# Nuralamsiddik16/Ultrafnd_git

Hardware: AMD Instinct MI355X
Metric: train-step samples/sec (FakeSV batch, seq128+224^2) (higher is better)
Workload: dtype bf16

## Files before the change

### ultrafnd_git_amd/csrc/gemm_bf16_kernel.hpp

```cpp
#pragma once
#ifndef UFND_GEMM_OUT_NT
#define UFND_GEMM_OUT_NT 0
#endif

#include <type_traits>

#include "common.hpp"
#include "attn_softmax.hpp"

#pragma clang fp contract(off)

#ifndef UFND_GEMM_ILV
#define UFND_GEMM_ILV 1
#endif

namespace {

constexpr int BK = 64;

struct GemmArgs {
  const __bf16* A;
  const __bf16* W;
  const float* bias;
  const float* residual;
  __bf16* out_bf16;
  float* out_f32;
  int M, N, K, lda, ldw, ldr, ldo, ldf, act;
  int m_tiles, n_tiles;
  unsigned long long* stamps;
  const float* a_stats;
  const float* colsum;
  const float* r_stats;
  const float* r_gamma;
  const float* r_beta;
  float* out_stats;
  int a_parts, r_parts;
  float a_eps, r_eps, inv_h;
  const int32_t* att_mask;
  __bf16* att_ctx;
  int att_h;
  int xcd_cols;
  float att_scale_log2e;
  const __bf16* residual_b;
  int ldrb;
  int ksplit;
  size_t slab_stride;
  const __bf16* aux;
  int ldaux;
  float* guard;
  int pp_rows;
  const int* m_live;
  const int32_t* att_cu;
  const int32_t* att_bins;
  const int* att_nbins;
};

__device__ __forceinline__ void dma16(const void* gsrc, void* lds_dst) {
  __builtin_amdgcn_global_load_lds((const void __attribute__((address_space(1)))*)gsrc,
                                   (void __attribute__((address_space(3)))*)lds_dst, 16, 0, 0);
}

__device__ __forceinline__ float opaque_f(float x) {
  asm volatile("" : "+v"(x));
  return x;
}
__device__ __forceinline__ f32x2 opaque_f2(f32x2 x) {
  asm volatile("" : "+v"(x));
  return x;
}

__device__ __forceinline__ bf16x8 lds_frag(const char* tile, int row, int chunk) {
  return *reinterpret_cast<const bf16x8*>(tile + row * 128 + ((chunk ^ ((row >> 1) & 7)) << 4));
}

template <int N>
__device__ __forceinline__ void wait_vmcnt() {
  static_assert(N >= 0 && N <= 63, "vmcnt range");
  asm volatile("s_waitcnt vmcnt(%0)" ::"n"(N) : "memory");
}

template <int V> struct IntC { static constexpr int value = V; };

constexpr int gemm_waves_per_simd(int BM, int BN, int WM, int WN, int STA, int STB, int MI, int LNX, int ATT) {
  const int ring = (STA * BM + STB * BN) * 128, cbytes = WM * WN * MI * (BN / WN + 4) * 4;
  const int smem = (ring > cbytes ? ring : cbytes) + (LNX ? BM * 8 + 64 : 0);
  return (!ATT && smem <= 80 * 1024 ? 2 : 1) * WM * WN / 4;
}
template <int BM, int BN, int WM, int WN, int STA, int STB, int MI, int ABL = 0, int DBG = 0, int LNX = 0, int ATT = 0, int BWD = 0>
__global__ __launch_bounds__(WM * WN * 64) __attribute__((amdgpu_waves_per_eu(gemm_waves_per_simd(BM, BN, WM, WN, STA, STB, MI, LNX, ATT))))
void gemm_bf16_kernel(const GemmArgs a) {
  static_assert(!BWD || (!LNX && !ATT && !ABL && !DBG), "backward forms are plain kernels");
  static_assert(MI == 16 || MI == 32, "MFMA shape");
  static_assert(!ATT || (BM == 128 && BN == 384 && MI == 16 && WM * WN == 8 && LNX == 1), "fused attention tile");
  using acc_t = typename std::conditional<MI == 16, f32x4, f32x16>::type;
  constexpr int AR = MI * MI / 64;
  constexpr int KQ = MI == 16 ? 1 : 2;
  constexpr int NW = WM * WN;
  constexpr int TM = BM / WM, TN = BN / WN;
  constexpr int MT = TM / MI, NT = TN / MI;
  constexpr int ASLOT = BM * 128, BSLOT = BN * 128;
  constexpr int DA = STA - 1, DB = STB - 1;
  constexpr int APIECES = BM / 8, BPIECES = BN / 8;
  constexpr int PWA = APIECES / NW, PWB = (BPIECES + NW - 1) / NW;
  constexpr int WAITN = PWA * (DA - 1 > 0 ? DA - 1 : 0) + PWB * (DB - 1 > 0 ? DB - 1 : 0);
  constexpr int CP = TN + 4;
  constexpr int CBYTES = NW * MI * CP * 4;
  constexpr int RING = STA * ASLOT + STB * BSLOT;
  constexpr int ATT_OFF = (CBYTES + 1023) & ~1023;
  constexpr int ATT_END = ATT ? ATT_OFF + 6 * 16384 + 2048 : 0;
  constexpr int STAT_OFF0 = (RING > CBYTES) ? RING : CBYTES;
  constexpr int STAT_OFF = STAT_OFF0 > ATT_END ? STAT_OFF0 : ATT_END;
  constexpr int SMEM = STAT_OFF + (LNX ? BM * 8 + 64 : 0);
  static_assert(SMEM <= 160 * 1024, "LDS budget");
  static_assert(APIECES % NW == 0 && TM % MI == 0 && TN % MI == 0, "tile split");
  static_assert(STB >= 2 && (STA == STB || STA == STB + 1), "ring depths");
  static_assert(WAITN <= 63, "vmcnt range");
  __shared__ __attribute__((aligned(16))) char smem[SMEM];

  unsigned long long stamp[10];
  if constexpr (DBG) {
    stamp[0] = __builtin_amdgcn_s_memtime();
    stamp[1] = __builtin_amdgcn_s_memrealtime();
  }

  int mlive = a.M, m_tiles = a.m_tiles;
  if constexpr (!BWD && !ATT) {
    if (a.m_live) {
      const int v = __builtin_amdgcn_readfirstlane(*a.m_live);
      mlive = v < a.M ? (v > 0 ? v : 0) : a.M;
      m_tiles = (mlive + BM - 1) / BM;
      if ((int)blockIdx.x >= m_tiles * a.n_tiles) return;
    }
  }
  if constexpr (ATT) {
    if (a.att_bins) {
      const int v = __builtin_amdgcn_readfirstlane(*a.att_nbins);
      m_tiles = v < a.m_tiles ? (v > 0 ? v : 0) : a.m_tiles;
      if ((int)blockIdx.x >= m_tiles * a.n_tiles) return;
    }
  }
  const int nblk = m_tiles * a.n_tiles;
  int bid, kslice = 0;
  {
    const int ngrid = BWD ? nblk * (a.ksplit > 1 ? a.ksplit : 1) : nblk;
    const int q = ngrid >> 3, r = ngrid & 7, xcd = blockIdx.x & 7, idx = blockIdx.x >> 3;
    bid = (xcd < r ? xcd * (q + 1) : r * (q + 1) + (xcd - r) * q) + idx;
    if constexpr (BWD) {
      kslice = bid / nblk;
      bid -= kslice * nblk;
    }
  }
  int tm = bid / a.n_tiles, tn = bid % a.n_tiles;
  if (a.xcd_cols == 2) {
    const int nh = a.n_tiles >> 1, per_half = m_tiles * nh;
    const int half = bid / per_half, rem = bid - half * per_half;
    tm = rem / nh;
    tn = half * nh + (rem - tm * nh);
  }
  const int m0 = tm * BM, n0 = tn * BN;
  int arow0 = m0, alen = BM;
  int srow[4] = {0, 0, 0, 0}, scnt[4] = {0, 0, 0, 0}, smeta[4] = {-1, -1, -1, -1};
  const bool slots = ATT && a.att_bins != nullptr;
  if constexpr (ATT) {
    if (slots) {
      const int32_t* bd = a.att_bins + (size_t)tm * 8;
#pragma unroll
      for (int j = 0; j < 4; ++j) {
        srow[j] = __builtin_amdgcn_readfirstlane(bd[2 * j]);
        smeta[j] = __builtin_amdgcn_readfirstlane(bd[2 * j + 1]);
        const int n = smeta[j] & 255, rest = n - 32 * ((smeta[j] >> 8) & 3);
        scnt[j] = smeta[j] < 0 ? 0 : (rest < 32 ? rest : 32);
      }
#pragma unroll
      for (int j = 1; j < 4; ++j) srow[j] = scnt[j] > 0 ? srow[j] : srow[0];
    } else if (a.att_cu) {
      mlive = __builtin_amdgcn_readfirstlane(*a.m_live);
      arow0 = __builtin_amdgcn_readfirstlane(a.att_cu[tm]);
      alen = __builtin_amdgcn_readfirstlane(a.att_cu[tm + 1]) - arow0;
      if (alen <= 0) return;
    }
  } else {
    alen = mlive - m0;
  }
  auto tile_row = [&](int tr) {
    if (slots) {
      const int j = tr >> 5, q = tr & 31;
      const int r0 = j == 0 ? srow[0] : j == 1 ? srow[1] : j == 2 ? srow[2] : srow[3];
      const int c = j == 0 ? scnt[0] : j == 1 ? scnt[1] : j == 2 ? scnt[2] : scnt[3];
      return r0 + (q < c ? q : (c > 0 ? c - 1 : 0));
    }
    const int gr = arow0 + tr;
    return gr < mlive ? gr : mlive - 1;
  };
  auto tile_row_live = [&](int tr) {
    if (slots) {
      const int j = tr >> 5;
      return (tr & 31) < (j == 0 ? scnt[0] : j == 1 ? scnt[1] : j == 2 ? scnt[2] : scnt[3]);
    }
    return tr < alen;
  };
  const int wave = __builtin_amdgcn_readfirstlane(threadIdx.x >> 6), lane = threadIdx.x & 63;
  const int wm = wave / WN, wn = wave % WN, fr = lane & (MI - 1), g = lane / MI;

  acc_t acc[MT][NT];
#pragma unroll
  for (int i = 0; i < MT; ++i)
#pragma unroll
    for (int j = 0; j < NT; ++j)
#pragma unroll
      for (int r = 0; r < AR; ++r) acc[i][j][r] = 0.f;

  int nk = a.K / BK, kbase = 0;
  if constexpr (BWD) {
    if (a.ksplit > 1) {
      const int per = (nk + a.ksplit - 1) / a.ksplit;
      kbase = kslice * per * BK;
      nk = nk - kslice * per < per ? nk - kslice * per : per;
    }
  }
  const int prow = lane >> 3, ppos = lane & 7;
  int arow_att[ATT ? PWA : 1];
  if constexpr (ATT) {
#pragma unroll
    for (int ii = 0; ii < PWA; ++ii) arow_att[ii] = tile_row(8 * (wave + NW * ii) + prow);
  }
  auto issueA = [&](int t, int kt) {
    char* buf = smem + (t % STA) * ASLOT;
    const int k0 = kbase + kt * BK;
#pragma unroll
    for (int ii = 0; ii < PWA; ++ii) {
      const int p = wave + NW * ii;
      const int r = 8 * p + prow;
      const int c = ppos ^ ((r >> 1) & 7);
      int gr = arow0 + r;
      gr = gr < mlive ? gr : mlive - 1;
      if constexpr (ATT) gr = arow_att[ii];
      dma16(a.A + (size_t)gr * a.lda + k0 + c * 8, buf + p * 1024);
    }
  };
  auto issueB = [&](int t, int kt) {
    char* buf = smem + STA * ASLOT + (t % STB) * BSLOT;
    const int k0 = kbase + kt * BK;
#pragma unroll
    for (int ii = 0; ii < PWB; ++ii) {
      int p = wave + NW * ii;
      if constexpr (BPIECES % NW != 0) p = p < BPIECES ? p : p - BPIECES;
      const int r = 8 * p + prow;
      const int c = ppos ^ ((r >> 1) & 7);
      int gr = n0 + r;
      gr = gr < a.N ? gr : a.N - 1;
      if constexpr (ATT) gr = (r >> 7) * a.att_h + tn * 128 + (r & 127);
      dma16(a.W + (size_t)gr * a.ldw + k0 + c * 8, buf + p * 1024);
    }
  };
  constexpr int TPR = NW * 64 / BM;
  static_assert(!LNX || TPR == 2 || TPR == 4, "threads per tile row");
  constexpr int GPT = 4 / (TPR < 4 ? TPR : 4);
  f32x4 sv[GPT][3];
  f32x2* st_lds = reinterpret_cast<f32x2*>(smem + STAT_OFF);
  const float* sp = nullptr;
  if constexpr (LNX) {
    sp = a.a_stats ? a.a_stats : a.r_stats;
    if (sp) {
      const int parts = a.a_stats ? a.a_parts : a.r_parts;
      int row = arow0 + (int)threadIdx.x / TPR;
      row = row < mlive ? row : mlive - 1;
      if constexpr (ATT) row = tile_row((int)threadIdx.x / TPR);
      const f32x4* base = reinterpret_cast<const f32x4*>(sp + (size_t)row * parts * 2);
      const int nq = parts >> 1, sub = threadIdx.x % TPR;
#pragma unroll
      for (int gi = 0; gi < GPT; ++gi)
#pragma unroll
        for (int u = 0; u < 3; ++u) {
          const int q = (sub + gi * TPR) + 4 * u;
          asm volatile("global_load_dwordx4 %0, %1, off" : "=v"(sv[gi][u]) : "v"(base + (q < nq ? q : 0)) : "memory");
        }
    }
  }
  int att_mk = 1;
  if constexpr (ATT) {
    if (slots) {
      const int j = (int)threadIdx.x >> 7, k = threadIdx.x & 127;
      const int mt = j == 0 ? smeta[0] : j == 1 ? smeta[1] : j == 2 ? smeta[2] : smeta[3];
      att_mk = mt >= 0 && k < (mt & 255);
      if (att_mk && a.att_mask) att_mk = a.att_mask[(size_t)(mt >> 10) * BM + k];
    } else if (a.att_mask && threadIdx.x < BM) {
      att_mk = a.att_mask[m0 + threadIdx.x];
    }
  }
#pragma unroll
  for (int s = 0; s < STA; ++s) {
    const int ks = s < nk ? s : nk - 1;
    if (s < STB && (LNX || s < nk)) issueB(s, ks);
    if (LNX || s < nk) issueA(s, ks);
  }

  if constexpr (LNX) {
    if (sp) {
      constexpr int NPRO = STA * PWA + STB * PWB;
      static_assert(NPRO <= 63, "vmcnt range");
      if constexpr (GPT == 1)
        asm volatile("s_waitcnt vmcnt(%3) ; STATRETIRE %0 %1 %2" : "+v"(sv[0][0]), "+v"(sv[0][1]), "+v"(sv[0][2]) : "n"(NPRO) : "memory");
      else
        asm volatile("s_waitcnt vmcnt(%6) ; STATRETIRE %0 %1 %2 %3 %4 %5" : "+v"(sv[0][0]), "+v"(sv[0][1]), "+v"(sv[0][2]), "+v"(sv[GPT - 1][0]),
                     "+v"(sv[GPT - 1][1]), "+v"(sv[GPT - 1][2]) : "n"(NPRO) : "memory");
      const int nq_ = (a.a_stats ? a.a_parts : a.r_parts) >> 1, sub_ = threadIdx.x % TPR;
      float gs[GPT], gq[GPT];
#pragma unroll
      for (int gi = 0; gi < GPT; ++gi) {
#pragma unroll
        for (int u = 0; u < 3; ++u) {
          if ((sub_ + gi * TPR) + 4 * u >= nq_) sv[gi][u] = f32x4{0.f, 0.f, 0.f, 0.f};
        }
        gs[gi] = sv[gi][0][0] + sv[gi][0][2];
        gq[gi] = sv[gi][0][1] + sv[gi][0][3];
#pragma unroll
        for (int u = 1; u < 3; ++u) { gs[gi] += sv[gi][u][0] + sv[gi][u][2]; gq[gi] += sv[gi][u][1] + sv[gi][u][3]; }
      }
      float sm, sq;
      if constexpr (TPR == 4) {
        sm = gs[0] + quad_xor1(gs[0]);
        sq = gq[0] + quad_xor1(gq[0]);
        sm += quad_xor2(sm);
        sq += quad_xor2(sq);
      } else {
        const float s01 = gs[0] + quad_xor1(gs[0]), s23 = gs[1] + quad_xor1(gs[1]);
        const float q01 = gq[0] + quad_xor1(gq[0]), q23 = gq[1] + quad_xor1(gq[1]);
        sm = s01 + s23;
        sq = q01 + q23;
      }
      const float mean = __fmul_rn(sm, a.inv_h);
      const float var = fmaxf(__fmaf_rn(-mean, mean, __fmul_rn(sq, a.inv_h)), 0.f);
      const float rstd = __builtin_amdgcn_rsqf(__fadd_rn(var, a.a_stats ? a.a_eps : a.r_eps));
      if (threadIdx.x % TPR == 0) st_lds[threadIdx.x / TPR] = f32x2{mean, rstd};
      if (a.guard && a.a_stats) {
        float ratio = __fmul_rn(fabsf(mean), rstd);
        ratio = ratio == ratio ? ratio : INFINITY;
        const float worst = wave_max(threadIdx.x % TPR == 0 && tile_row_live((int)threadIdx.x / TPR) ? ratio : 0.0f);
        if (lane == 0) reinterpret_cast<float*>(smem + STAT_OFF + BM * 8)[wave] = worst;
      }
      asm volatile("s_waitcnt lgkmcnt(0)" ::: "memory");
    }
  }

  bf16x8 af0[KQ][MT], bf0[KQ][NT], af1[KQ][MT], bf1[KQ][NT];
  auto read_half = [&](int t, auto kk_, bf16x8 (&af)[KQ][MT], bf16x8 (&bfr)[KQ][NT]) {
    constexpr int kk = decltype(kk_)::value;
    const char* At = smem + (t % STA) * ASLOT;
    const char* Bt = smem + STA * ASLOT + (t % STB) * BSLOT;
#pragma unroll
    for (int q = 0; q < KQ; ++q) {
      const int chunk = MI == 16 ? g + 4 * kk : g + 2 * q + 4 * kk;
#pragma unroll
      for (int i = 0; i < MT; ++i) af[q][i] = lds_frag(At, wm * TM + i * MI + fr, chunk);
#pragma unroll
      for (int j = 0; j < NT; ++j) bfr[q][j] = lds_frag(Bt, wn * TN + j * MI + fr, chunk);
    }
  };
  auto mma_half = [&](const bf16x8 (&af)[KQ][MT], const bf16x8 (&bfr)[KQ][NT]) {
#pragma unroll
    for (int q = 0; q < KQ; ++q)
#pragma unroll
      for (int i = 0; i < MT; ++i)
#pragma unroll
        for (int j = 0; j < NT; ++j) {
          if constexpr (MI == 16) acc[i][j] = __builtin_amdgcn_mfma_f32_16x16x32_bf16(af[q][i], bfr[q][j], acc[i][j], 0, 0, 0);
          else acc[i][j] = __builtin_amdgcn_mfma_f32_32x32x16_bf16(af[q][i], bfr[q][j], acc[i][j], 0, 0, 0);
        }
  };
  constexpr int NMF = KQ * MT * NT, NRD = KQ * (MT + NT);
  constexpr bool ILV = UFND_GEMM_ILV != 0;
  auto body = [&](int t, auto ia_, auto ib_, auto next_) {
    constexpr bool IA = decltype(ia_)::value != 0, IB = decltype(ib_)::value != 0, NEXT = decltype(next_)::value != 0;
    if constexpr (ABL != 1) {
      read_half(t, IntC<1>{}, af1, bf1);
      mma_half(af0, bf0);
      if constexpr (ILV) {
#pragma unroll
        for (int q = 0; q < (NRD < NMF ? NRD : NMF - 1); ++q) {
          __builtin_amdgcn_sched_group_barrier(0x008, 1, 0);
          __builtin_amdgcn_sched_group_barrier(0x100, 1, 0);
        }
        __builtin_amdgcn_sched_group_barrier(0x100, NRD - (NRD < NMF ? NRD : NMF - 1), 0);
        __builtin_amdgcn_sched_group_barrier(0x008, NMF - (NRD < NMF ? NRD : NMF - 1), 0);
      } else {
        __builtin_amdgcn_sched_group_barrier(0x008, 1, 0);
        __builtin_amdgcn_sched_group_barrier(0x100, NRD, 0);
        __builtin_amdgcn_sched_group_barrier(0x008, NMF - 1, 0);
      }
    }
    if constexpr (NEXT) {
      __builtin_amdgcn_sched_barrier(0);
      if (t + STA - 1 < nk) wait_vmcnt<WAITN>();
      else wait_vmcnt<0>();
      asm volatile("s_waitcnt lgkmcnt(0)" ::: "memory");
      __builtin_amdgcn_s_barrier();
      __builtin_amdgcn_sched_barrier(0);
      if constexpr (ABL != 1) read_half(t + 1, IntC<0>{}, af0, bf0);
      if constexpr (ABL != 2) {
        if constexpr (IB) issueB(t + STB, t + STB);
        if constexpr (IA) issueA(t + STA, t + STA);
      }
    }
    if constexpr (ABL != 1) {
      mma_half(af1, bf1);
      constexpr int PW = (ABL == 2 || !NEXT) ? 0 : (IA ? PWA : 0) + (IB ? PWB : 0);
      constexpr int GRP = (NMF - 1) / (PW + 1) > 0 ? (NMF - 1) / (PW + 1) : 1;
      if constexpr (ILV && NEXT && NRD + PW < NMF) {
#pragma unroll
        for (int q = 0; q < NRD; ++q) {
          __builtin_amdgcn_sched_group_barrier(0x008, 1, 0);
          __builtin_amdgcn_sched_group_barrier(0x100, 1, 0);
        }
        constexpr int REST = NMF - NRD, G2 = REST / (PW + 1) > 0 ? REST / (PW + 1) : 1;
#pragma unroll
        for (int q = 0; q < PW; ++q) {
          __builtin_amdgcn_sched_group_barrier(0x008, G2, 0);
          __builtin_amdgcn_sched_group_barrier(0x020, 1, 0);
        }
        __builtin_amdgcn_sched_group_barrier(0x008, REST - G2 * PW > 0 ? REST - G2 * PW : 0, 0);
      } else {
        __builtin_amdgcn_sched_group_barrier(0x008, 1, 0);
        if constexpr (NEXT) __builtin_amdgcn_sched_group_barrier(0x100, NRD, 0);
#pragma unroll
        for (int q = 0; q < PW; ++q) {
          __builtin_amdgcn_sched_group_barrier(0x008, GRP, 0);
          __builtin_amdgcn_sched_group_barrier(0x020, 1, 0);
        }
        __builtin_amdgcn_sched_group_barrier(0x008, NMF - 1 - GRP * PW > 0 ? NMF - 1 - GRP * PW : 0, 0);
      }
    }
  };

  if (STA <= nk) wait_vmcnt<PWA * (STA - 1) + PWB * (STB - 1)>();
  else wait_vmcnt<0>();
  __builtin_amdgcn_sched_barrier(0);
  __builtin_amdgcn_s_barrier();
  __builtin_amdgcn_sched_barrier(0);
  if constexpr (DBG) {
    stamp[2] = __builtin_amdgcn_s_memtime();
    stamp[3] = __builtin_amdgcn_s_memrealtime();
  }
  if constexpr (ABL != 1) read_half(0, IntC<0>{}, af0, bf0);
  int t = 0;
  for (; t + STA < nk; ++t) body(t, IntC<1>{}, IntC<1>{}, IntC<1>{});
  for (; t + STB < nk; ++t) body(t, IntC<0>{}, IntC<1>{}, IntC<1>{});
  for (; t + 1 < nk; ++t) body(t, IntC<0>{}, IntC<0>{}, IntC<1>{});
  body(t, IntC<0>{}, IntC<0>{}, IntC<0>{});
  __builtin_amdgcn_sched_barrier(0);
  __builtin_amdgcn_s_barrier();
  __builtin_amdgcn_sched_barrier(0);
  if constexpr (DBG) {
    stamp[4] = __builtin_amdgcn_s_memtime();
    stamp[5] = __builtin_amdgcn_s_memrealtime();
  }

  float bj[NT], csj[NT];
#pragma unroll
  for (int j = 0; j < NT; ++j) { bj[j] = 0.f; csj[j] = 0.f; }
  auto gcol = [&](int c) { return ATT ? (c >> 7) * a.att_h + tn * 128 + (c & 127) : n0 + c; };
  if (a.bias) {
#pragma unroll
    for (int j = 0; j < NT; ++j) bj[j] = a.bias[gcol(wn * TN + j * MI + fr)];
  }
  bool fold = false, rln = false;
  if constexpr (LNX) {
    fold = a.a_stats != nullptr;
    rln = a.r_stats != nullptr;
    if (fold) {
#pragma unroll
      for (int j = 0; j < NT; ++j) csj[j] = a.colsum[gcol(wn * TN + j * MI + fr)];
    }
  }
  float* cst = reinterpret_cast<float*>(smem) + wave * MI * CP;
  float* const outf = (BWD && a.out_f32) ? a.out_f32 + (size_t)kslice * a.slab_stride : a.out_f32;
  constexpr int CPR = TN / 8;
  constexpr int CHUNKS = MI * CPR;
  constexpr int NIT = (CHUNKS + 63) / 64;
  constexpr bool FIXCOL = (64 % CPR) == 0;
  auto ld8 = [&](const float* ptr, float (&o)[8]) {
    const f32x4 x0 = *reinterpret_cast<const f32x4*>(ptr), x1 = *reinterpret_cast<const f32x4*>(ptr + 4);
#pragma unroll
    for (int q = 0; q < 4; ++q) { o[q] = x0[q]; o[4 + q] = x1[q]; }
  };
  float g8[8], b8[8];
  if constexpr (LNX && FIXCOL) {
    if (rln) {
      const int col = n0 + wn * TN + (lane % CPR) * 8;
      ld8(a.r_gamma + col, g8);
      ld8(a.r_beta + col, b8);
    }
  }
  auto epilogue = [&](auto act_, auto mode_) {
    constexpr int ACT = decltype(act_)::value;
    constexpr bool FOLD = LNX && decltype(mode_)::value == 1, RLN = LNX && decltype(mode_)::value == 2;
    constexpr bool RES = !FOLD;
#pragma unroll
    for (int i = 0; i < MT; ++i) {
      float rr8[RES ? NIT : 1][8];
      if constexpr (RES) if (a.residual && !(BWD && a.aux)) {
#pragma unroll
        for (int it = 0; it < NIT; ++it) {
          const int id = lane + 64 * it;
          if (id < CHUNKS) {
            int row = m0 + wm * TM + i * MI + id / CPR;
            row = row < a.M ? row : a.M - 1;
            ld8(a.residual + (size_t)row * a.ldr + n0 + wn * TN + (id % CPR) * 8, rr8[it]);
          }
        }
      }
      if constexpr (BWD) {
        if (a.aux) {
#pragma unroll
          for (int it = 0; it < NIT; ++it) {
            const int id = lane + 64 * it;
            if (id < CHUNKS) {
              int row = m0 + wm * TM + i * MI + id / CPR;
              row = row < a.M ? row : a.M - 1;
              const bf16x8 xb = *reinterpret_cast<const bf16x8*>(a.aux + (size_t)row * a.ldaux + n0 + wn * TN + (id % CPR) * 8);
#pragma unroll
              for (int q = 0; q < 8; ++q) rr8[it][q] = (float)xb[q];
            }
          }
        }
      }
      if constexpr (LNX && RES) {
        if (a.residual_b) {
#pragma unroll
          for (int it = 0; it < NIT; ++it) {
            const int id = lane + 64 * it;
            if (id < CHUNKS) {
              int row = m0 + wm * TM + i * MI + id / CPR;
              row = row < a.M ? row : a.M - 1;
              const bf16x8 rb = *reinterpret_cast<const bf16x8*>(a.residual_b + (size_t)row * a.ldrb + n0 + wn * TN + (id % CPR) * 8);
#pragma unroll
              for (int q = 0; q < 8; ++q) rr8[it][q] = (float)rb[q];
            }
          }
        }
      }
#pragma unroll
      for (int r = 0; r < AR; r += 2) {
        const int prow_ = MI == 16 ? 4 * g + r : 8 * (r >> 2) + 4 * g + (r & 3);
        f32x2 mean2 = {0.f, 0.f}, rstd2 = {1.f, 1.f};
        if constexpr (FOLD) {
          const f32x2 a0 = st_lds[wm * TM + i * MI + prow_], a1 = st_lds[wm * TM + i * MI + prow_ + 1];
          mean2 = f32x2{a0[0], a1[0]};
          rstd2 = f32x2{a0[1], a1[1]};
        }
#pragma unroll
        for (int j = 0; j < NT; ++j) {
          f32x2 v = {acc[i][j][r], acc[i][j][r + 1]};
          if constexpr (FOLD) v = opaque_f2(rstd2 * __builtin_elementwise_fma(-mean2, f32x2{csj[j], csj[j]}, v));
          v = v + f32x2{bj[j], bj[j]};
          if constexpr (ACT == UFND_ACT_GELU) v = gelu_fast_f2(v);
          else if constexpr (ACT == UFND_ACT_QUICK_GELU) v = quick_gelu_fast_f2(v);
          cst[prow_ * CP + j * MI + fr] = v.x;
          cst[(prow_ + 1) * CP + j * MI + fr] = v.y;
        }
      }
      asm volatile("s_waitcnt lgkmcnt(0)" ::: "memory");
#pragma unroll
      for (int it = 0; it < NIT; ++it) {
        const int id = lane + 64 * it;
        if (id >= CHUNKS) break;
        const int rr = id / CPR, cl = (id % CPR) * 8;
        const int row = m0 + wm * TM + i * MI + rr;
        const int col = n0 + wn * TN + cl;
        const bool live = row < mlive;
        const f32x4 v0 = *reinterpret_cast<const f32x4*>(cst + rr * CP + cl);
        const f32x4 v1 = *reinterpret_cast<const f32x4*>(cst + rr * CP + cl + 4);
        float v[8] = {v0[0], v0[1], v0[2], v0[3], v1[0], v1[1], v1[2], v1[3]};
        if constexpr (BWD) {
          if (a.aux) {
            if (a.act == UFND_ACT_GELU_BWD) {
#pragma unroll
              for (int q = 0; q < 8; ++q) v[q] = v[q] * gelu_grad_f(rr8[it][q]);
            } else {
#pragma unroll
              for (int q = 0; q < 8; ++q) v[q] = v[q] * quick_gelu_grad_f(rr8[it][q]);
            }
          }
        }
        if constexpr (RES) if ((a.residual && !(BWD && a.aux)) || (LNX && a.residual_b)) {
          if constexpr (RLN) {
            const f32x2 ms = st_lds[wm * TM + i * MI + rr];
            if constexpr (!FIXCOL) {
              ld8(a.r_gamma + col, g8);
              ld8(a.r_beta + col, b8);
            }
#pragma unroll
            for (int q = 0; q < 8; ++q) rr8[it][q] = __fmaf_rn(__fmul_rn(__fsub_rn(rr8[it][q], ms[0]), ms[1]), g8[q], b8[q]);
          }
#pragma unroll
          for (int q = 0; q < 8; ++q) v[q] = __fadd_rn(v[q], rr8[it][q]);
        }
        if constexpr (LNX && RES) {
          if (a.out_stats) {
            if constexpr (CPR % 4 == 0) {
              float sm = 0.f, sq = 0.f;
#pragma unroll
              for (int q = 0; q < 8; ++q) { sm = __fadd_rn(sm, v[q]); sq = __fmaf_rn(v[q], v[q], sq); }
              sm += quad_xor1(sm);
              sq += quad_xor1(sq);
              sm += quad_xor2(sm);
              sq += quad_xor2(sq);
              if (live && (id & 3) == 0)
                *reinterpret_cast<f32x2*>(a.out_stats + ((size_t)row * (a.N >> 5) + (col >> 5)) * 2) = f32x2{sm, sq};
            }
          }
        }
        if constexpr (ATT) {
          const int ct = wn * TN + cl;
          const int trow = wm * TM + i * MI + rr, img = ct >> 6, ch = (ct & 63) >> 3;
          bf16x8 o;
#pragma unroll
          for (int q = 0; q < 8; ++q) o[q] = (__bf16)v[q];
          const int sw = img >= 4 ? (ch ^ (((trow >> 1) & 3) << 1)) : (ch ^ ((trow >> 1) & 7));
          *reinterpret_cast<bf16x8*>(smem + ATT_OFF + img * 16384 + trow * 128 + (sw << 4)) = o;
          continue;
        }
        if (!live) continue;
        if (a.out_f32) {
          float* op = outf + (size_t)row * a.ldf + col;
          *reinterpret_cast<f32x4*>(op) = f32x4{v[0], v[1], v[2], v[3]};
          *reinterpret_cast<f32x4*>(op + 4) = f32x4{v[4], v[5], v[6], v[7]};
        }
        if (a.out_bf16) {
          bf16x8 o;
#pragma unroll
          for (int q = 0; q < 8; ++q) o[q] = (__bf16)v[q];
          if constexpr (UFND_GEMM_OUT_NT && !BWD) __builtin_nontemporal_store(o, reinterpret_cast<bf16x8*>(a.out_bf16 + (size_t)row * a.ldo + col));
          else *reinterpret_cast<bf16x8*>(a.out_bf16 + (size_t)row * a.ldo + col) = o;
        }
      }
      asm volatile("s_waitcnt lgkmcnt(0)" ::: "memory");
    }
  };
  if constexpr (LNX) {
    if (fold) {
      if (a.act == UFND_ACT_GELU) epilogue(IntC<UFND_ACT_GELU>{}, IntC<1>{});
      else if (a.act == UFND_ACT_QUICK_GELU) epilogue(IntC<UFND_ACT_QUICK_GELU>{}, IntC<1>{});
      else epilogue(IntC<UFND_ACT_NONE>{}, IntC<1>{});
    } else if (rln) {
      epilogue(IntC<UFND_ACT_NONE>{}, IntC<2>{});
    } else {
      epilogue(IntC<UFND_ACT_NONE>{}, IntC<0>{});
    }
  } else {
    if (a.act == UFND_ACT_GELU) epilogue(IntC<UFND_ACT_GELU>{}, IntC<0>{});
    else if (a.act == UFND_ACT_QUICK_GELU) epilogue(IntC<UFND_ACT_QUICK_GELU>{}, IntC<0>{});
    else epilogue(IntC<UFND_ACT_NONE>{}, IntC<0>{});
  }
  if constexpr (ATT && DBG) {
    stamp[8] = __builtin_amdgcn_s_memtime();
    stamp[9] = __builtin_amdgcn_s_memrealtime();
  }
  if constexpr (ATT) {
    constexpr float NEG_MASK = -3.0e38f;
    float* kbias = reinterpret_cast<float*>(smem + ATT_OFF + 6 * 16384);
    if (slots || threadIdx.x < BM) kbias[threadIdx.x] = att_mk != 0 ? 0.0f : NEG_MASK;
    __syncthreads();
    const int hh = wave >> 2, wq = wave & 3, g4 = lane >> 4, f16 = lane & 15;
    int wrow0 = arow0 + 32 * wq, wcnt = alen - 32 * wq, koff = 0;
    const float* wbias = kbias;
    if (slots) {
      const int mt = wq == 0 ? smeta[0] : wq == 1 ? smeta[1] : wq == 2 ? smeta[2] : smeta[3];
      wrow0 = wq == 0 ? srow[0] : wq == 1 ? srow[1] : wq == 2 ? srow[2] : srow[3];
      wcnt = wq == 0 ? scnt[0] : wq == 1 ? scnt[1] : wq == 2 ? scnt[2] : scnt[3];
      koff = 32 * (wq - ((mt >> 8) & 3));
      wbias = kbias + wq * BM;
    }
    const char* qimg = smem + ATT_OFF + hh * 16384;
    const char* kimg = smem + ATT_OFF + (2 + hh) * 16384;
    const char* vimg = smem + ATT_OFF + (4 + hh) * 16384;
    bf16x8 qf[2][2];
#pragma unroll
    for (int qt = 0; qt < 2; ++qt) {
      const int q = wq * 32 + qt * 16 + f16;
      qf[qt][0] = lds_frag(qimg, q, g4);
      qf[qt][1] = lds_frag(qimg, q, g4 + 4);
    }
    f32x4 o[4][2];
#pragma unroll
    for (int dt = 0; dt < 4; ++dt)
#pragma unroll
      for (int qt = 0; qt < 2; ++qt) o[dt][qt] = f32x4{0.f, 0.f, 0.f, 0.f};
    float m_run[2] = {-INFINITY, -INFINITY}, l_run[2] = {0.f, 0.f};
    constexpr int KB = 64, KT = KB / 16;
    if (wcnt > 0) {
#pragma unroll
    for (int kb0 = 0; kb0 < BM; kb0 += KB) {
      const int kr0 = koff + kb0;
      if (masked_block_is_noop(wbias + kb0, lane, m_run)) continue;
      f32x4 sc[KT][2];
#pragma unroll
      for (int kt = 0; kt < KT; ++kt)
#pragma unroll
        for (int qt = 0; qt < 2; ++qt) sc[kt][qt] = f32x4{0.f, 0.f, 0.f, 0.f};
#pragma unroll
      for (int kk = 0; kk < 2; ++kk)
#pragma unroll
        for (int kt = 0; kt < KT; ++kt) {
          const bf16x8 kf = lds_frag(kimg, (kr0 + kt * 16 + f16) & (BM - 1), g4 + 4 * kk);
#pragma unroll
          for (int qt = 0; qt < 2; ++qt) sc[kt][qt] = __builtin_amdgcn_mfma_f32_16x16x32_bf16(kf, qf[qt][kk], sc[kt][qt], 0, 0, 0);
        }
      const bool any_masked = __any(wbias[kb0 + lane] != 0.0f);
      bf16x8 pf[KT / 2][2];
#pragma unroll
      for (int qt = 0; qt < 2; ++qt) {
        const float alpha = online_softmax_block<KT>(sc, qt, wbias + kb0, any_masked, g4, a.att_scale_log2e, m_run[qt], l_run[qt], pf);
        if (!__all(alpha == 1.0f)) {
#pragma unroll
          for (int dt = 0; dt < 4; ++dt) o[dt][qt] *= alpha;
        }
      }
#pragma unroll
      for (int ksd = 0; ksd < KT / 2; ++ksd) {
#pragma unroll
        for (int dt = 0; dt < 4; ++dt) {
          const int qq = f16 >> 2, pp = f16 & 3;
          const int key0 = (kr0 + 32 * ksd + 4 * g4 + qq) & (BM - 1);
          const int ch = 2 * dt + (pp >> 1);
          const int off0 = key0 * 128 + ((ch ^ (((key0 >> 1) & 3) << 1)) << 4) + 8 * (pp & 1);
          const int key1 = key0 + 16;
          const int off1 = key1 * 128 + ((ch ^ (((key1 >> 1) & 3) << 1)) << 4) + 8 * (pp & 1);
          const s16x4 t0 = __builtin_amdgcn_ds_read_tr16_b64_v4i16((s16x4 __attribute__((address_space(3)))*)(vimg + off0));
          const s16x4 t1 = __builtin_amdgcn_ds_read_tr16_b64_v4i16((s16x4 __attribute__((address_space(3)))*)(vimg + off1));
          union { s16x4 s2[2]; bf16x8 v; } u;
          u.s2[0] = t0;
          u.s2[1] = t1;
#pragma unroll
          for (int qt = 0; qt < 2; ++qt) o[dt][qt] = __builtin_amdgcn_mfma_f32_16x16x32_bf16(u.v, pf[ksd][qt], o[dt][qt], 0, 0, 0);
        }
      }
    }
    }
#pragma unroll
    for (int qt = 0; qt < 2; ++qt) {
      float l = l_run[qt];
      l += __shfl_xor(l, 16, 64);
      l += __shfl_xor(l, 32, 64);
      const float inv = 1.0f / l;
      const int q = qt * 16 + f16;
      if (q >= wcnt) continue;
      __bf16* dst = a.att_ctx + (size_t)(wrow0 + q) * a.att_h + (tn * 2 + hh) * 64 + 4 * g4;
#pragma unroll
      for (int dt = 0; dt < 4; ++dt) {
        bf16x4 ov = {(__bf16)(o[dt][qt][0] * inv), (__bf16)(o[dt][qt][1] * inv), (__bf16)(o[dt][qt][2] * inv), (__bf16)(o[dt][qt][3] * inv)};
        *reinterpret_cast<bf16x4*>(dst + dt * 16) = ov;
      }
    }
  }
  if constexpr (LNX) {
    if (a.guard && a.a_stats && threadIdx.x == 0) {
      const float* gw = reinterpret_cast<const float*>(smem + STAT_OFF + BM * 8);
      float worst = gw[0];
#pragma unroll
      for (int w = 1; w < NW; ++w) worst = fmaxf(worst, gw[w]);
      atomicMax(reinterpret_cast<int*>(a.guard + (blockIdx.x & 1023)), __float_as_int(worst));
    }
  }
  if constexpr (DBG) {
    asm volatile("s_waitcnt vmcnt(0)" ::: "memory");
    stamp[6] = __builtin_amdgcn_s_memtime();
    stamp[7] = __builtin_amdgcn_s_memrealtime();
    if (threadIdx.x == 0) {
      constexpr int NS = ATT ? 10 : 8;
#pragma unroll
      for (int i = 0; i < NS; ++i) a.stamps[(size_t)blockIdx.x * NS + i] = stamp[i];
    }
  }
}

}

#define UFND_GEMM_TILES(X)                                                                             \
  X(0, 128, 128, 2, 2, 3, 3, 16, 0, 0)                                                              \
  X(1, 128, 64, 2, 2, 3, 3, 16, 0, 0)                                                 \
  X(2, 256, 128, 4, 2, 3, 3, 16, 1, 1)                                                              \
  X(3, 128, 128, 2, 2, 2, 2, 16, 1, 0)                                                \
  X(4, 128, 64, 2, 2, 4, 4, 16, 0, 0)                                                               \
  X(5, 256, 64, 4, 2, 3, 3, 16, 0, 0)                                                               \
  X(6, 128, 288, 2, 2, 3, 3, 16, 0, 0)                                   \
  X(7, 128, 96, 2, 2, 3, 3, 16, 0, 0)                                     \
  X(8, 256, 192, 4, 2, 2, 2, 16, 1, 1)                                  \
  X(9, 128, 384, 2, 2, 2, 2, 16, 0, 0)                                                              \
  X(10, 128, 192, 2, 2, 3, 3, 16, 0, 0)                                                             \
  X(11, 128, 96, 2, 2, 4, 4, 16, 0, 0)                                                              \
  X(12, 64, 96, 1, 2, 4, 4, 16, 0, 0)                     \
  X(13, 64, 192, 1, 2, 3, 3, 16, 0, 0)                                                              \
  X(14, 128, 256, 2, 2, 2, 2, 16, 0, 0)                                                             \
  X(15, 256, 256, 4, 2, 2, 2, 16, 1, 1)                                                             \
  X(16, 128, 128, 4, 2, 3, 3, 16, 1, 1)                                  \
  X(17, 128, 192, 4, 2, 3, 3, 16, 1, 1)                                  \
  X(18, 256, 64, 4, 2, 4, 4, 16, 0, 0)                                                              \
  X(19, 64, 64, 1, 2, 4, 4, 16, 0, 0)                                                 \
  X(20, 128, 64, 4, 2, 4, 4, 16, 1, 1)                                   \
  X(21, 256, 192, 2, 4, 2, 2, 16, 0, 0)                                          \
  X(22, 256, 192, 4, 2, 3, 2, 16, 1, 1)                                 \
  X(23, 256, 256, 4, 2, 3, 2, 16, 0, 0)                                                             \
  X(24, 128, 192, 4, 2, 4, 4, 16, 0, 0)                                                             \
  X(25, 128, 256, 4, 2, 3, 3, 16, 0, 0)                                 \
  X(26, 256, 192, 4, 2, 2, 2, 32, 0, 0)   \
  X(27, 128, 128, 4, 2, 3, 3, 32, 0, 0)                                                                    \
  X(28, 256, 144, 8, 1, 2, 2, 16, 1, 1)   \
  X(29, 128, 128, 4, 2, 2, 2, 16, 1, 0)

#ifdef UFND_DIAG
#define UFND_TILE_BUILT(PROD_) 1
#else
#define UFND_TILE_BUILT(PROD_) (PROD_)
#endif

struct TileCfg { int bm, bn, threads, wn, lnx, built; };
static const TileCfg kTiles[] = {
#define X(id, BM_, BN_, WM_, WN_, SA_, SB_, MI_, LN_, PROD_) {BM_, BN_, WM_ * WN_ * 64, WN_, LN_, UFND_TILE_BUILT(PROD_)},
    UFND_GEMM_TILES(X)
#undef X
};
constexpr int kNumTiles = sizeof(kTiles) / sizeof(kTiles[0]);

static int xcd_cols_for(int M, int N, int K, int m_tiles, int n_tiles) {
#ifdef UFND_DIAG
  static const int forced = [] { const char* e = getenv("UFND_GEMM_XCD_COLS"); return e ? atoi(e) : 0; }();
  if (forced == 1) return 1;
  if (forced == 2) return (n_tiles % 2 == 0) ? 2 : 1;
#endif
  (void)K;
  return (4LL * N > (long long)M && n_tiles % 2 == 0 && m_tiles >= 4) ? 2 : 1;
}

static int launch_cfg(int cfg, int mode, GemmArgs& a, hipStream_t stream) {
  if (cfg < 0 || cfg >= kNumTiles || !kTiles[cfg].built) {
    ufnd_set_error("gemm_bf16: tile config %d is not part of this library", cfg);
    return UFND_ERR_INVALID;
  }
  const TileCfg& t = kTiles[cfg];
  a.m_tiles = ufnd_cdiv(a.M, t.bm);
  a.n_tiles = a.N / t.bn;
  a.xcd_cols = xcd_cols_for(a.M, a.N, a.K, a.m_tiles, a.n_tiles);
  const dim3 grid(a.m_tiles * a.n_tiles * (mode == 6 && a.ksplit > 1 ? a.ksplit : 1)), block(t.threads);
#ifdef UFND_GEMM_ONLY_BWD
#define X(id, BM_, BN_, WM_, WN_, SA_, SB_, MI_, LN_, PROD_)                                                                      \
  case id:                                                                                                                        \
    if constexpr (id == 15 || id == 16 || id == 17 || id == 20 || id == 22) {                                                     \
      hipLaunchKernelGGL((gemm_bf16_kernel<BM_, BN_, WM_, WN_, SA_, SB_, MI_, 0, 0, 0, 0, 1>), grid, block, 0, stream, a);        \
    } else {                                                                                                                      \
      ufnd_set_error("gemm_bf16 backward: tile %d has no backward kernel", id);                                                   \
      return UFND_ERR_INVALID;                                                                                                    \
    }                                                                                                                             \
    break;
  (void)mode;
  switch (cfg) {
    UFND_GEMM_TILES(X)
    default: ufnd_set_error("gemm_bf16: unknown tile config %d", cfg); return UFND_ERR_INVALID;
  }
#undef X
  return UFND_OK;
#else
#ifdef UFND_DIAG
#define UFND_DIAG_LAUNCH(BM_, BN_, WM_, WN_, SA_, SB_, MI_)                                                                             \
  else if (mode == 5) hipLaunchKernelGGL((gemm_bf16_kernel<BM_, BN_, WM_, WN_, SA_, SB_, MI_, 0, 1, 1>), grid, block, 0, stream, a);   \
  else if (mode == 1) hipLaunchKernelGGL((gemm_bf16_kernel<BM_, BN_, WM_, WN_, SA_, SB_, MI_, 1, 0>), grid, block, 0, stream, a);      \
  else if (mode == 2) hipLaunchKernelGGL((gemm_bf16_kernel<BM_, BN_, WM_, WN_, SA_, SB_, MI_, 2, 0>), grid, block, 0, stream, a);      \
  else if (mode == 3) hipLaunchKernelGGL((gemm_bf16_kernel<BM_, BN_, WM_, WN_, SA_, SB_, MI_, 0, 1>), grid, block, 0, stream, a);
#else
#define UFND_DIAG_LAUNCH(BM_, BN_, WM_, WN_, SA_, SB_, MI_)
#endif
#define X(id, BM_, BN_, WM_, WN_, SA_, SB_, MI_, LN_, PROD_)                                                        \
  case id:                                                                                                          \
    if constexpr (UFND_TILE_BUILT(PROD_) != 0) {                                                                    \
      if (mode == 0) {                                                                                              \
        hipLaunchKernelGGL((gemm_bf16_kernel<BM_, BN_, WM_, WN_, SA_, SB_, MI_, 0, 0>), grid, block, 0, stream, a); \
      } else if constexpr (LN_ != 0) {    \
        if (mode == 4) hipLaunchKernelGGL((gemm_bf16_kernel<BM_, BN_, WM_, WN_, SA_, SB_, MI_, 0, 0, 1>), grid, block, 0, stream, a); \
        UFND_DIAG_LAUNCH(BM_, BN_, WM_, WN_, SA_, SB_, MI_)                                                         \
        else {                                                                                                      \
          ufnd_set_error("gemm_bf16: tile %d has no kernel for mode %d in this library", id, mode);                 \
          return UFND_ERR_INVALID;                                                                                  \
        }                                                                                                           \
      } else {                                                                                                      \
        ufnd_set_error("gemm_bf16: tile %d has no diagnostics / LayerNorm-aware build", id);                        \
        return UFND_ERR_INVALID;                                                                                    \
      }                                                                                                             \
    }                                                                                                               \
    break;
  switch (cfg) {
    UFND_GEMM_TILES(X)
    default: ufnd_set_error("gemm_bf16: unknown tile config %d", cfg); return UFND_ERR_INVALID;
  }
#undef X
#undef UFND_DIAG_LAUNCH
  return UFND_OK;
#endif
}

static int auto_cfg(int M, int N, int K) {
#ifdef UFND_DIAG
  static const int forced = [] { const char* e = getenv("UFND_GEMM_FORCE_CFG"); return e ? atoi(e) : -1; }();
  if (forced >= 0 && forced < kNumTiles && N % kTiles[forced].bn == 0) return forced;
#endif
  auto tiles = [&](int cfg) { return (long long)ufnd_cdiv(M, kTiles[cfg].bm) * (N / kTiles[cfg].bn); };
  if (N % 256 == 0 && N >= 3072 && tiles(15) >= 512) return 15;
  if (N % 256 == 0 && N >= 2048 && tiles(15) >= 190 && tiles(15) <= 256) return 15;
  if (N % 192 == 0 && tiles(22) >= 160) return 22;
  if (N >= 2048) {
    if (N % 192 == 0 && N >= 3072) return 17;
    if (N % 128 == 0) return 16;
  }
  if (N < 2048 && N % 192 == 0 && tiles(17) >= 150 && tiles(17) <= 256) return 17;
  if (N % 128 == 0 && tiles(16) >= 150) return 16;
  return 20;
}
```

Measured before the change: 29020.

## Write fused-attention QKV tiles from registers with V stored transposed in LDS

For the fused attention tile, the QKV GEMM epilogue now writes Q/K directly from MFMA accumulators (using swapped operand order so rows are contiguous) and stores V pre-transposed into a dedicated LDS image, instead of staging through the generic per-wave C buffer. The P·V loop then reads V fragments with plain 128-bit LDS loads instead of two ds_read_tr16 transposing reads per fragment. Column mapping per wave is changed so each wave owns head-aligned slices, and the attention region now overlaps the start of LDS. This removes a staging pass and the transpose-read cost but changes layout invariants in several places, with risk of aliasing the staging/ring regions.

```diff
diff --git a/ultrafnd_git_amd/csrc/gemm_bf16_kernel.hpp b/ultrafnd_git_amd/csrc/gemm_bf16_kernel.hpp
--- a/ultrafnd_git_amd/csrc/gemm_bf16_kernel.hpp
+++ b/ultrafnd_git_amd/csrc/gemm_bf16_kernel.hpp
@@ -106,7 +106,7 @@
   constexpr int CP = TN + 4;
   constexpr int CBYTES = NW * MI * CP * 4;
   constexpr int RING = STA * ASLOT + STB * BSLOT;
-  constexpr int ATT_OFF = (CBYTES + 1023) & ~1023;
+  constexpr int ATT_OFF = 0;
   constexpr int ATT_END = ATT ? ATT_OFF + 6 * 16384 + 2048 : 0;
   constexpr int STAT_OFF0 = (RING > CBYTES) ? RING : CBYTES;
   constexpr int STAT_OFF = STAT_OFF0 > ATT_END ? STAT_OFF0 : ATT_END;
@@ -202,6 +202,7 @@
   const int wave = __builtin_amdgcn_readfirstlane(threadIdx.x >> 6), lane = threadIdx.x & 63;
   const int wm = wave / WN, wn = wave % WN, fr = lane & (MI - 1), g = lane / MI;
 
+  auto wcol = [&](int j) { return ATT ? (j >> 1) * 128 + (2 * wn + (j & 1)) * MI : wn * TN + j * MI; };
   acc_t acc[MT][NT];
 #pragma unroll
   for (int i = 0; i < MT; ++i)
@@ -354,7 +355,7 @@
 #pragma unroll
       for (int i = 0; i < MT; ++i) af[q][i] = lds_frag(At, wm * TM + i * MI + fr, chunk);
 #pragma unroll
-      for (int j = 0; j < NT; ++j) bfr[q][j] = lds_frag(Bt, wn * TN + j * MI + fr, chunk);
+      for (int j = 0; j < NT; ++j) bfr[q][j] = lds_frag(Bt, wcol(j) + fr, chunk);
     }
   };
   auto mma_half = [&](const bf16x8 (&af)[KQ][MT], const bf16x8 (&bfr)[KQ][NT]) {
@@ -364,7 +365,10 @@
       for (int i = 0; i < MT; ++i)
 #pragma unroll
         for (int j = 0; j < NT; ++j) {
-          if constexpr (MI == 16) acc[i][j] = __builtin_amdgcn_mfma_f32_16x16x32_bf16(af[q][i], bfr[q][j], acc[i][j], 0, 0, 0);
+          if constexpr (ATT) {
+            if (j < 4) acc[i][j] = __builtin_amdgcn_mfma_f32_16x16x32_bf16(bfr[q][j], af[q][i], acc[i][j], 0, 0, 0);
+            else acc[i][j] = __builtin_amdgcn_mfma_f32_16x16x32_bf16(af[q][i], bfr[q][j], acc[i][j], 0, 0, 0);
+          } else if constexpr (MI == 16) acc[i][j] = __builtin_amdgcn_mfma_f32_16x16x32_bf16(af[q][i], bfr[q][j], acc[i][j], 0, 0, 0);
           else acc[i][j] = __builtin_amdgcn_mfma_f32_32x32x16_bf16(af[q][i], bfr[q][j], acc[i][j], 0, 0, 0);
         }
   };
@@ -459,7 +463,7 @@
 #pragma unroll
   for (int j = 0; j < NT; ++j) { bj[j] = 0.f; csj[j] = 0.f; }
   auto gcol = [&](int c) { return ATT ? (c >> 7) * a.att_h + tn * 128 + (c & 127) : n0 + c; };
-  if (a.bias) {
+  if (!ATT && a.bias) {
 #pragma unroll
     for (int j = 0; j < NT; ++j) bj[j] = a.bias[gcol(wn * TN + j * MI + fr)];
   }
@@ -467,7 +471,7 @@
   if constexpr (LNX) {
     fold = a.a_stats != nullptr;
     rln = a.r_stats != nullptr;
-    if (fold) {
+    if (!ATT && fold) {
 #pragma unroll
       for (int j = 0; j < NT; ++j) csj[j] = a.colsum[gcol(wn * TN + j * MI + fr)];
     }
@@ -610,16 +614,6 @@
             }
           }
         }
-        if constexpr (ATT) {
-          const int ct = wn * TN + cl;
-          const int trow = wm * TM + i * MI + rr, img = ct >> 6, ch = (ct & 63) >> 3;
-          bf16x8 o;
-#pragma unroll
-          for (int q = 0; q < 8; ++q) o[q] = (__bf16)v[q];
-          const int sw = img >= 4 ? (ch ^ (((trow >> 1) & 3) << 1)) : (ch ^ ((trow >> 1) & 7));
-          *reinterpret_cast<bf16x8*>(smem + ATT_OFF + img * 16384 + trow * 128 + (sw << 4)) = o;
-          continue;
-        }
         if (!live) continue;
         if (a.out_f32) {
           float* op = outf + (size_t)row * a.ldf + col;
@@ -637,7 +631,77 @@
       asm volatile("s_waitcnt lgkmcnt(0)" ::: "memory");
     }
   };
-  if constexpr (LNX) {
+  auto att_epilogue = [&](auto fold_) {
+    constexpr bool FOLD = decltype(fold_)::value != 0;
+    const int head = wn >> 1, dt0 = 2 * (wn & 1);
+    f32x4 b4[4], c4[4];
+    float bv[2], cv[2];
+#pragma unroll
+    for (int j = 0; j < 4; ++j) {
+      const int col = gcol(wcol(j) + 4 * g);
+      b4[j] = a.bias ? *reinterpret_cast<const f32x4*>(a.bias + col) : f32x4{0.f, 0.f, 0.f, 0.f};
+      c4[j] = f32x4{0.f, 0.f, 0.f, 0.f};
+      if constexpr (FOLD) c4[j] = *reinterpret_cast<const f32x4*>(a.colsum + col);
+    }
+#pragma unroll
+    for (int j = 0; j < 2; ++j) {
+      const int col = gcol(wcol(4 + j) + fr);
+      bv[j] = a.bias ? a.bias[col] : 0.f;
+      cv[j] = 0.f;
+      if constexpr (FOLD) cv[j] = a.colsum[col];
+    }
+#pragma unroll
+    for (int i = 0; i < MT; ++i) {
+      const int trow = wm * TM + i * MI + fr;
+      f32x2 mean2 = {0.f, 0.f}, rstd2 = {1.f, 1.f};
+      if constexpr (FOLD) {
+        const f32x2 ms = st_lds[trow];
+        mean2 = f32x2{ms[0], ms[0]};
+        rstd2 = f32x2{ms[1], ms[1]};
+      }
+#pragma unroll
+      for (int j = 0; j < 4; ++j) {
+        bf16x4 o;
+#pragma unroll
+        for (int r = 0; r < 4; r += 2) {
+          f32x2 v = {acc[i][j][r], acc[i][j][r + 1]};
+          if constexpr (FOLD) v = opaque_f2(rstd2 * __builtin_elementwise_fma(-mean2, f32x2{c4[j][r], c4[j][r + 1]}, v));
+          v = v + f32x2{b4[j][r], b4[j][r + 1]};
+          o[r] = (__bf16)v.x;
+          o[r + 1] = (__bf16)v.y;
+        }
+        const int img = (j >> 1) * 2 + head, ch = 2 * (dt0 + (j & 1)) + (g >> 1);
+        *reinterpret_cast<bf16x4*>(smem + ATT_OFF + img * 16384 + trow * 128 + ((ch ^ ((trow >> 1) & 7)) << 4) + 8 * (g & 1)) = o;
+      }
+    }
+#pragma unroll
+    for (int i = 0; i < MT; i += 2) {
+#pragma unroll
+      for (int j = 0; j < 2; ++j) {
+        bf16x8 o;
+#pragma unroll
+        for (int ii = 0; ii < 2; ++ii)
+#pragma unroll
+          for (int r = 0; r < 4; r += 2) {
+            f32x2 v = {acc[i + ii][4 + j][r], acc[i + ii][4 + j][r + 1]};
+            if constexpr (FOLD) {
+              const int t0 = wm * TM + (i + ii) * MI + 4 * g + r;
+              const f32x2 a0 = st_lds[t0], a1 = st_lds[t0 + 1];
+              v = opaque_f2(f32x2{a0[1], a1[1]} * __builtin_elementwise_fma(-f32x2{a0[0], a1[0]}, f32x2{cv[j], cv[j]}, v));
+            }
+            v = v + f32x2{bv[j], bv[j]};
+            o[4 * ii + r] = (__bf16)v.x;
+            o[4 * ii + r + 1] = (__bf16)v.y;
+          }
+        const int d = (dt0 + j) * MI + fr, ch = 4 * (wm * (TM / 32) + (i >> 1)) + g;
+        *reinterpret_cast<bf16x8*>(smem + ATT_OFF + (4 + head) * 16384 + d * 256 + ((ch ^ fr) << 4)) = o;
+      }
+    }
+  };
+  if constexpr (ATT) {
+    if (fold) att_epilogue(IntC<1>{});
+    else att_epilogue(IntC<0>{});
+  } else if constexpr (LNX) {
     if (fold) {
       if (a.act == UFND_ACT_GELU) epilogue(IntC<UFND_ACT_GELU>{}, IntC<1>{});
       else if (a.act == UFND_ACT_QUICK_GELU) epilogue(IntC<UFND_ACT_QUICK_GELU>{}, IntC<1>{});
@@ -720,19 +784,10 @@
       for (int ksd = 0; ksd < KT / 2; ++ksd) {
 #pragma unroll
         for (int dt = 0; dt < 4; ++dt) {
-          const int qq = f16 >> 2, pp = f16 & 3;
-          const int key0 = (kr0 + 32 * ksd + 4 * g4 + qq) & (BM - 1);
-          const int ch = 2 * dt + (pp >> 1);
-          const int off0 = key0 * 128 + ((ch ^ (((key0 >> 1) & 3) << 1)) << 4) + 8 * (pp & 1);
-          const int key1 = key0 + 16;
-          const int off1 = key1 * 128 + ((ch ^ (((key1 >> 1) & 3) << 1)) << 4) + 8 * (pp & 1);
-          const s16x4 t0 = __builtin_amdgcn_ds_read_tr16_b64_v4i16((s16x4 __attribute__((address_space(3)))*)(vimg + off0));
-          const s16x4 t1 = __builtin_amdgcn_ds_read_tr16_b64_v4i16((s16x4 __attribute__((address_space(3)))*)(vimg + off1));
-          union { s16x4 s2[2]; bf16x8 v; } u;
-          u.s2[0] = t0;
-          u.s2[1] = t1;
-#pragma unroll
-          for (int qt = 0; qt < 2; ++qt) o[dt][qt] = __builtin_amdgcn_mfma_f32_16x16x32_bf16(u.v, pf[ksd][qt], o[dt][qt], 0, 0, 0);
+          const int ch = 4 * (((kr0 >> 5) + ksd) & 3) + g4;
+          const bf16x8 vf = *reinterpret_cast<const bf16x8*>(vimg + (dt * 16 + f16) * 256 + ((ch ^ f16) << 4));
+#pragma unroll
+          for (int qt = 0; qt < 2; ++qt) o[dt][qt] = __builtin_amdgcn_mfma_f32_16x16x32_bf16(vf, pf[ksd][qt], o[dt][qt], 0, 0, 0);
         }
       }
     }
```

Measured after the change: 29240 (median of 6 runs). Within noise of the previous version (+0.8%).
